# 0beqz/realism-effects

Hardware: AMD Instinct MI355X
Metric: Mpixels/s SSGI+denoise @4K steps=20; achieved HBM GB/s vs peak (higher is better)
Workload: dtype f32; 1 GPU; configs[2]: 3840x2160 (8.29 Mpixel) on one GPU, steps=20 refineSteps=5 denoiseIterations=1, K1+K2+2xK3+K4 per step; frame=3840x2160, tile_rows=2160, halo_rows=0, direct_light=True, half_store=rtz, uv_model=reference_gl, parallelism=single GPU

## Files before the change

realism-effects_amd/csrc/k1_ssgi.hip:

```cpp
#include "rfx_blocks.h"
#include "rfx_brdf.h"
#include "rfx_kernels.h"
#include "rfx_launch.h"

namespace {

constexpr int BASE = 16;
constexpr int K1_TH = 1;
typedef uint32_t k1_cell_t;
constexpr int K1_WAVES = 8;
constexpr int K1_COUNTERS = 64;
constexpr int K1_TABLE_CELLS = RFX_K1_TABLE_BYTES / (int)sizeof(k1_cell_t);
RFX_DEV uint32_t k1_half_toward(float v, bool up) {
    uint32_t h = rfx_f2h_rne(v) & 0xffffu;
    const float f = rfx_h2f((unsigned short)h);
    if (up ? (f < v) : (f > v)) {
        const bool neg = (h & 0x8000u) != 0;
        if (up) h = neg ? (h == 0x8000u ? 0x0001u : h - 1u) : h + 1u;
        else h = neg ? h + 1u : (h == 0x0000u ? 0x8001u : h - 1u);
    }
    return h;
}
RFX_DEV k1_cell_t k1_cell_pack(float mn, float mx) { return k1_half_toward(mn, false) | (k1_half_toward(mx, true) << 16); }
RFX_DEV float2 k1_cell_load(const k1_cell_t *t, unsigned int i) {
    const uint32_t v = *(const k1_cell_t *)((const char *)t + i);
    return make_float2(rfx_h2f((unsigned short)(v & 0xffffu)), rfx_h2f((unsigned short)(v >> 16)));
}

struct MarchCtx {
    const float *P;
    const float *viewz;
    const k1_cell_t *coarse;
    int coarse_w, cell_shift;
    unsigned int cell_xmask;
    int cell_xshift, cell_yshift;
    float rayDistance, thickness;
    int steps, refineSteps;
};

RFX_DEV float k1_div(float x, float w, float r) {
    const float q = x * r;
    return __builtin_fmaf(__builtin_fmaf(-w, q, x), r, q);
}
constexpr int PROJ_GENERAL = 0, PROJ_PERSPECTIVE = 1, PROJ_CENTRED = 2;
constexpr int PROJ_TABLE_POW2 = 4;
constexpr int k1_proj_kind(int proj) { return proj & 3; }
constexpr bool k1_table_pow2(int proj) { return (proj & PROJ_TABLE_POW2) != 0; }
template <int PROJ_T>
RFX_DEV float2 k1_project(const MarchCtx &m, float3 p) {
    constexpr int PROJ = k1_proj_kind(PROJ_T);
    float px, py, pw;
    if (PROJ == PROJ_CENTRED) {
        px = m.P[0] * p.x;
        py = m.P[5] * p.y;
        pw = -p.z;
    } else if (PROJ == PROJ_PERSPECTIVE) {
        px = m.P[0] * p.x + m.P[8] * p.z;
        py = m.P[5] * p.y + m.P[9] * p.z;
        pw = -p.z;
    } else {
        const float4 pc = rfx_mat_mul(m.P, p.x, p.y, p.z, 1.0f);
        px = pc.x; py = pc.y; pw = pc.w;
    }
    const float r = rfx_rcp(pw);
    return make_float2(__builtin_fmaf(k1_div(px, pw, r), 0.5f, 0.5f), __builtin_fmaf(k1_div(py, pw, r), 0.5f, 0.5f));
}

struct Tap {
    unsigned int idx;
    unsigned int cell;
};
template <bool P2>
RFX_DEV Tap k1_tap_at(const MarchCtx &m, const FrameDims &d, int xi, int yi) {
    Tap t;
    t.idx = (unsigned int)(__mul24(yi, d.W) + xi);
    if (P2) {
        const unsigned int a = (unsigned int)xi >> m.cell_xshift, b = (unsigned int)yi << m.cell_yshift;
        t.cell = (unsigned int)__builtin_amdgcn_bitop3_b32((int)a, (int)b, (int)m.cell_xmask, 0xE4);
    } else {
// ... 55 lines not shown
    if (need[0] | need[1]) {
        const unsigned int i0 = need[0] ? tap[0].idx : tap[1].idx, i1 = need[1] ? tap[1].idx : tap[0].idx;
        const float z0 = rfx_gather<float>(m.viewz, i0), z1 = rfx_gather<float>(m.viewz, i1);
        const float d0 = z0 - rays[0].pos.z, d1 = z1 - rays[1].pos.z;
        rays[0].live = (need[0] & (d0 >= 0.0f) & (d0 < m.thickness)) ? 0.0f : rays[0].live;
        rays[1].live = (need[1] & (d1 >= 0.0f) & (d1 < m.thickness)) ? 0.0f : rays[1].live;
    }
}
template <int PROJ>
RFX_DEV void k1_refine_pairs(const MarchCtx &m, const FrameDims &d, Ray (&rays)[2]) {
#pragma unroll
    for (int r = 0; r < 2; r++) {
        rays[r].dir = rays[r].dir * 0.5f;
        rays[r].pos = rays[r].pos + rays[r].dir * (rays[r].hit ? -1.0f : 0.0f);
    }
    for (int k = 0; k < m.refineSteps; k++) {
#pragma unroll
        for (int r = 0; r < 2; r++)
            if (rays[r].hit) rays[r].uv = k1_project<PROJ>(m, rays[r].pos);
        Tap tap[2];
        float2 mm[2];
        bool need[2], behind[2];
#pragma unroll
        for (int r = 0; r < 2; r++) tap[r] = k1_tap<k1_table_pow2(PROJ)>(m, d, rays[r].uv);
#pragma unroll
        for (int r = 0; r < 2; r++) {
            need[r] = rays[r].hit;
            behind[r] = false;
        }
#pragma unroll
        for (int r = 0; r < 2; r++) mm[r] = k1_cell_load(m.coarse, tap[r].cell);
#pragma unroll
        for (int r = 0; r < 2; r++) {
            const float h = rays[r].pos.z;
            const bool below = mm[r].y - h < 0.0f;
            const bool above = !below & (mm[r].x - h >= 0.0f);
            need[r] = need[r] & !(below | above);
            behind[r] = above;
        }
        float z[2];
#pragma unroll
        for (int r = 0; r < 2; r++) z[r] = need[r] ? rfx_gather<float>(m.viewz, tap[r].idx) : 0.0f;
#pragma unroll
        for (int r = 0; r < 2; r++) {
            if (need[r]) behind[r] = z[r] - rays[r].pos.z >= 0.0f;
            rays[r].dir = rays[r].dir * 0.5f;
            rays[r].pos = rays[r].pos + rays[r].dir * (rays[r].hit ? (behind[r] ? -1.0f : 1.0f) : 0.0f);
        }
    }
#pragma unroll
    for (int r = 0; r < 2; r++)
        if (rays[r].hit) rays[r].uv = k1_project<PROJ>(m, rays[r].pos);
}
RFX_DEV float k1_push(int dest_lane, float v) { return __int_as_float(__builtin_amdgcn_ds_permute(dest_lane << 2, __float_as_int(v))); }
RFX_DEV float k1_pull(int src_lane, float v) { return __int_as_float(__builtin_amdgcn_ds_bpermute(src_lane << 2, __float_as_int(v))); }
template <int PROJ>
RFX_DEV void k1_refine_packed(const MarchCtx &m, const FrameDims &d, Ray (&rays)[2], unsigned long long h0, unsigned long long h1, int n0, int n1) {
    const int lane = (int)__builtin_amdgcn_mbcnt_hi(~0u, __builtin_amdgcn_mbcnt_lo(~0u, 0u));
    const int rank0 = (int)__builtin_amdgcn_mbcnt_hi((unsigned int)(h0 >> 32), __builtin_amdgcn_mbcnt_lo((unsigned int)h0, 0u));
    const int rank1 = n0 + (int)__builtin_amdgcn_mbcnt_hi((unsigned int)(h1 >> 32), __builtin_amdgcn_mbcnt_lo((unsigned int)h1, 0u));
    const int dest0 = rays[0].hit ? rank0 : 63, dest1 = rays[1].hit ? rank1 : 63;
    const bool from0 = lane < n0, mine = lane < n0 + n1;
    float3 pos, dir;
#define K1_PACK(dst, field) { const float a = k1_push(dest0, rays[0].field), b = k1_push(dest1, rays[1].field); dst = from0 ? a : b; }
    K1_PACK(pos.x, pos.x) K1_PACK(pos.y, pos.y) K1_PACK(pos.z, pos.z) K1_PACK(dir.x, dir.x) K1_PACK(dir.y, dir.y) K1_PACK(dir.z, dir.z)
#undef K1_PACK
    dir = dir * 0.5f;
    pos = pos + dir * (mine ? -1.0f : 0.0f);
    float2 uv = make_float2(0.f, 0.f);
    for (int k = 0; k < m.refineSteps; k++) {
        if (mine) uv = k1_project<PROJ>(m, pos);
        const Tap tap = k1_tap<k1_table_pow2(PROJ)>(m, d, uv);
        const float2 mm = k1_cell_load(m.coarse, tap.cell);
        const float h = pos.z;
        const bool below = mm.y - h < 0.0f;
        const bool above = !below & (mm.x - h >= 0.0f);
        const bool need = mine & !(below | above);
        bool behind = above;
        const float z = need ? rfx_gather<float>(m.viewz, tap.idx) : 0.0f;
        if (need) behind = z - pos.z >= 0.0f;
        dir = dir * 0.5f;
        pos = pos + dir * (mine ? (behind ? -1.0f : 1.0f) : 0.0f);
    }
    if (mine) uv = k1_project<PROJ>(m, pos);
#define K1_UNPACK(val, f0, f1) { const float a = k1_pull(rank0, val), b = k1_pull(rank1, val); if (rays[0].hit) f0 = a; if (rays[1].hit) f1 = b; }
    K1_UNPACK(pos.x, rays[0].pos.x, rays[1].pos.x) K1_UNPACK(pos.y, rays[0].pos.y, rays[1].pos.y) K1_UNPACK(pos.z, rays[0].pos.z, rays[1].pos.z)
    K1_UNPACK(uv.x, rays[0].uv.x, rays[1].uv.x) K1_UNPACK(uv.y, rays[0].uv.y, rays[1].uv.y)
#undef K1_UNPACK
}
template <int PROJ>
RFX_DEV void k1_march_rays(const MarchCtx &m, const FrameDims &d, Ray (&rays)[2], float random_b) {
    const float scale = m.rayDistance / (float)m.steps;
    const bool started[2] = {rays[0].live != 0.0f, true};
#pragma unroll
    for (int r = 0; r < 2; r++) {
        rays[r].dir = rays[r].dir * scale;
        rays[r].uv = make_float2(0.f, 0.f);
    }
    const int split = min(m.steps, 9);
    int i = 1;
    for (; i < split && K1_ANY_LIVE(rays); i++) {
        const float t = (float)i + random_b - 0.5f;
        const float cs = 1.0f - rfx_exp2((t * t) * (-0.25f * 1.4426950408889634f));
        k1_march_step<PROJ, false>(m, d, rays, cs);
    }
    for (; i < m.steps && K1_ANY_LIVE(rays); i++) k1_march_step<PROJ, true>(m, d, rays, 1.0f);
#pragma unroll
    for (int r = 0; r < 2; r++) rays[r].hit = started[r] & (rays[r].live == 0.0f);
    if (m.refineSteps > 0) {
        const unsigned long long h0 = __ballot(rays[0].hit), h1 = __ballot(rays[1].hit);
        const int n0 = __popcll(h0), n1 = __popcll(h1);
// ... 267 lines not shown
        const float3 diffuseRay = (MIS && ems.isEnvSample) ? envMisDir : rfx_cosine_sample_hemisphere(viewNormal, rnd.x, rnd.y);
        diffuseRayDir = diffuseRay;
        const Angles ad = k1_angles(diffuseRay, vv, n);
        brdfD = k1_brdf_over_pdf_parts(mat, viewNormal, roughnessSq, true, NoV, ad, diffuseRay, pdfD);
        rays[0].dir = diffuseRay;
    }
    an = k1_angles(specularRay, vv, n);
    brdfS = k1_brdf_over_pdf_parts(mat, viewNormal, roughnessSq, isDiffuseSample, NoV, an, specularRay, pdfS);
    rays[1].live = 1.0f;
    rays[1].pos = viewPos;
    rays[1].dir = specularRay;
    if (STAGE == 2) {
        const float4 h0 = A.hits[2 * out_idx], h1 = A.hits[2 * out_idx + 1];
        rays[0].uv = make_float2(h0.x, h0.y);
        rays[1].uv = make_float2(h0.z, h0.w);
        rays[0].pos = make_float3(h1.x, h1.x, h1.x);
        rays[1].pos = make_float3(h1.y, h1.z, h1.w);
    } else {
        k1_march_rays<PROJ>(m, d, rays, rnd.z);
    }
    if (STAGE == 1) {
        A.hits[2 * out_idx] = make_float4(rays[0].uv.x, rays[0].uv.y, rays[1].uv.x, rays[1].uv.y);
        A.hits[2 * out_idx + 1] = make_float4(rays[0].pos.x, rays[1].pos.x, rays[1].pos.y, rays[1].pos.z);
        return;
    }

    float3 diffuseGI = make_float3(-1.0f, -1.0f, -1.0f);
    if (isDiffuseSample) diffuseGI = k1_shade<ENV, MIS>(d, A, mat, roughnessSq, rays[0], diffuseRayDir, true, brdfD, pdfD, ems) + dl;
    const float3 specularGI = k1_shade<ENV, MIS>(d, A, mat, roughnessSq, rays[1], specularRay, isDiffuseSample, brdfS, pdfS, ems) + dl;
    const float3 hitPos = rays[1].pos;

    float rayLength = 0.0f;
    if (!(hitPos.x > 10.0e8f)) {
        const float4 hw = rfx_mat_mul(C, hitPos.x, hitPos.y, hitPos.z, 1.0f);
        rayLength = rfx_length(make_float3(C[12], C[13], C[14]) - make_float3(hw.x, hw.y, hw.z));
    }
    if (p.mode == 0) {
        *outp = rfx_pack_two_vec4(make_float4(diffuseGI.x, diffuseGI.y, diffuseGI.z, mat.roughness),
                                  make_float4(specularGI.x, specularGI.y, specularGI.z, rayLength));
    } else {
        *outp = make_uint4(__float_as_uint(specularGI.x), __float_as_uint(specularGI.y), __float_as_uint(specularGI.z), rfx_pack_half2(rayLength, mat.roughness));
    }
}

template <int PROJ, bool ENV, bool MIS, int STAGE>
__global__ __launch_bounds__(64 * K1_WAVES) RFX_WAVES_PER_EU(ENV ? 1 : 8) void k1_ssgi_march(K1Args A) {
    __shared__ k1_cell_t s_cells[K1_TABLE_CELLS];
    if (STAGE != 2) {
        for (int i = threadIdx.x; i < A.cells_vec4; i += 64 * K1_WAVES) ((uint4 *)s_cells)[i] = ((const uint4 *)A.cells)[i];
        __syncthreads();
    }
    FrameDims d = A.dims;
    d.viol = 0;
    const int lane = threadIdx.x & 63;
    const unsigned int nbx = (unsigned int)(A.out_w + 63) / 64u, nby = (unsigned int)(A.y1 - A.y0 + K1_TH - 1) / (unsigned int)K1_TH, ntiles = nbx * nby;
    const unsigned int nq = min((unsigned int)K1_COUNTERS, gridDim.x);
    const unsigned int first = blockIdx.x % nq;
    unsigned int *counter = A.tile_counter + first * 32u;
    const auto k1_tile_of = [&](unsigned int n, unsigned int &bx, unsigned int &by) -> bool {
        const unsigned int tile = n * nq + first;
        by = tile / nbx;
        bx = tile - by * nbx;
        return tile < ntiles;
    };
    unsigned int n = 0;
    if (lane == 0) n = atomicAdd(counter, 1u);
    n = (unsigned int)__builtin_amdgcn_readfirstlane((int)n);
    unsigned int bx, by;
    while (k1_tile_of(n, bx, by)) {
        unsigned int next = 0;
        if (lane == 0) next = atomicAdd(counter, 1u);
        const int x = (int)bx * 64 + lane, y0 = A.y0 + (int)by * K1_TH;
#pragma unroll 1
        for (int r = 0; r < K1_TH; r++) {
            k1_ssgi_march_body<PROJ, ENV, MIS, STAGE>(RFX_KERNARGS_IN_LOOP(A), d, s_cells, x, y0 + r);
            RFX_WAVE_JOIN();
        }
        n = (unsigned int)__builtin_amdgcn_readfirstlane((int)next);
    }
    rfx_flush_violations(d);
}

__global__ __launch_bounds__(256) void k1_hit_mask(FrameDims d, int y0, int y1, TexView depth, TexViewW out, const float4 *hits, int allow_missed, unsigned int *mask) {
    const int x = blockIdx.x * 64 + threadIdx.x, y = y0 + blockIdx.y * 4 + threadIdx.y;
    d.viol = 0;
    if (x >= d.W || y >= y1) return;
    const float dp = ((const float *)depth.ptr)[rfx_xy_index(d, depth.row0, depth.rows, x, y)];
    if (dp == 1.0f) return;
    const size_t i = (size_t)rfx_local_row(d, out.row0, out.rows, y) * d.W + x;
    const float4 h0 = hits[2 * i], h1 = hits[2 * i + 1];
    const float u[2] = {h0.x, h0.z}, v[2] = {h0.y, h0.w}, px[2] = {h1.x, h1.y};
#pragma unroll
    for (int r = 0; r < 2; r++) {
        const bool missed = px[r] == 10.0e9f;
        if ((allow_missed || !missed) && u[r] >= 0.0f && u[r] <= 1.0f && v[r] >= 0.0f && v[r] <= 1.0f) {
            const int row = rfx_nearest_idx(v[r], d.fH, d.H), col = rfx_nearest_idx(u[r], d.fW, d.W);
            const unsigned int bit = 1u << rfx_block_of_col(col, d.W);
            if (!(mask[row] & bit)) atomicOr(&mask[row], bit);
        }
    }
}

template <int VEC>
__global__ __launch_bounds__(256) void k1_prepare(const float *depth, float *viewz, float2 *base, int W, int H, int base_w, float nearMulFar,
                                                   float farMinusNear, float cameraFar, float nearMinusFar, float cameraNear, int perspective,
                                                   unsigned char *fg, int fg_w) {
    static_assert(VEC == 1 || VEC == 4, "one texel or one aligned float4 per lane and row");
// ... 154 lines not shown
```

realism-effects_amd/csrc/k4_compose.hip:

```cpp
#include "k4_compose_texel.h"
#include "rfx_blocks.h"
#include "rfx_launch.h"

namespace {

template <bool WHOLE>
RFX_DEV void k4_compose_body(const K4Args &A, const FrameDims &d) {
    const int x = blockIdx.x * 64 + threadIdx.x;
    const int y = A.y0 + blockIdx.y * 4 + threadIdx.y;
    if (x >= d.W || y >= A.y1) return;
    const float u = rfx_frag_u(d.uv, x, y), v = rfx_frag_v(d.uv, y);
    const float *depthp = (const float *)A.depth.ptr;
    const float depth = depthp[rfx_xy_index(d, A.depth.row0, A.depth.rows, x, y)];
    {
        const int qx0 = x & ~1, qx1 = x | 1, qy0 = y & ~1, qy1 = y | 1;
        float dxa = depthp[rfx_xy_index(d, A.depth.row0, A.depth.rows, qx0, y)], dxb = depthp[rfx_xy_index(d, A.depth.row0, A.depth.rows, qx1, y)];
        float dya = depthp[rfx_xy_index(d, A.depth.row0, A.depth.rows, x, qy0)], dyb = depthp[rfx_xy_index(d, A.depth.row0, A.depth.rows, x, qy1)];
        if (depth == 1.0f && (fabsf(dxb - dxa) + fabsf(dyb - dya)) == 0.0f) {
            if (A.rgb_out) {
                const float4 keep = ((const float4 *)A.out.ptr)[(size_t)rfx_local_row(d, A.out.row0, A.out.rows, y) * d.W + x];
                float *r = A.rgb_out + ((size_t)y * d.W + x) * 3;
                r[0] = keep.x; r[1] = keep.y; r[2] = keep.z;
            }
            return;
        }
    }
    const Material mat = rfx_get_material<true>(((const uint4 *)A.gbuffer.ptr)[rfx_xy_index(d, A.gbuffer.row0, A.gbuffer.rows, x, y)]);
    float4 dgi = make_float4(0.f, 0.f, 0.f, 0.f), sgi;
    if (A.p.giSource) {
        const size_t gi = rfx_xy_index(d, A.gi0.row0, A.gi0.rows, x, y);
        if (A.p.inputType == 0) {
            dgi = ((const float4 *)A.gi0.ptr)[gi];
            sgi = ((const float4 *)A.gi1.ptr)[gi];
        } else {
            sgi = ((const float4 *)A.gi0.ptr)[gi];
        }
    } else if (A.p.inputType == 0) {
        dgi = rfx_fetch_h4_linear_fused<WHOLE>(A.gi0, d, u, v);
        sgi = rfx_fetch_h4_linear_fused<WHOLE>(A.gi1, d, u, v);
    } else {
        sgi = rfx_fetch_h4_linear_fused<WHOLE>(A.gi0, d, u, v);
    }
    float3 scene = make_float3(0.f, 0.f, 0.f);
    if (A.p.inputType == 2) {
        const float4 sc = ((const float4 *)A.scene.ptr)[rfx_xy_index(d, A.scene.row0, A.scene.rows, x, y)];
        scene = make_float3(sc.x, sc.y, sc.z);
    }
    const float4 o = k4_compose_texel(A.p, u, v, depth, mat, make_float3(dgi.x, dgi.y, dgi.z), make_float3(sgi.x, sgi.y, sgi.z), scene);
    ((float4 *)A.out.ptr)[(size_t)rfx_local_row(d, A.out.row0, A.out.rows, y) * d.W + x] = o;
    if (A.rgb_out) {
        float *r = A.rgb_out + ((size_t)y * d.W + x) * 3;
        r[0] = o.x; r[1] = o.y; r[2] = o.z;
    }
}

template <bool WHOLE>
__global__ __launch_bounds__(256) void k4_compose(K4Args A) {
    FrameDims d = A.dims;
    d.viol = 0;
    k4_compose_body<WHOLE>(A, d);
    rfx_flush_violations(d);
}

__global__ __launch_bounds__(256) void k5_final_compose(K5Args A) {
    FrameDims d = A.dims;
    d.viol = 0;
    const int x = blockIdx.x * 64 + threadIdx.x, y = A.y0 + blockIdx.y * 4 + threadIdx.y;
    if (x < d.W && y < A.y1) {
        const rfx_final_params &p = A.p;
        float4 o;
        const size_t gii = rfx_xy_index(d, A.gi.row0, A.gi.rows, x, y);
        const float4 gi = p.inputSource == 2 ? rfx_load_half4(((const uint2 *)A.gi.ptr)[gii]) : ((const float4 *)A.gi.ptr)[gii];
        if (p.isDebug) {
            o = gi;
        } else {
            const float depth = ((const float *)A.depth.ptr)[rfx_xy_index(d, A.depth.row0, A.depth.rows, x, y)];
            float3 c;
            if (depth == 1.0f) {
                const float4 sc = ((const float4 *)A.scene.ptr)[rfx_xy_index(d, A.scene.row0, A.scene.rows, x, y)];
                c = make_float3(sc.x, sc.y, sc.z);
            } else {
                c = make_float3(gi.x, gi.y, gi.z);
                if (p.fogMode) {
                    const float n_ = p.camera.near_, f_ = p.camera.far_;
                    const float viewZ = rfx_depth_to_view_z(depth, n_, f_, p.camera.isPerspective != 0) * 0.4f;
                    const float fd = -viewZ;
                    float ff;
                    if (p.fogMode == 2) {
                        ff = 1.0f - rfx_exp(((-p.fogDensity * p.fogDensity) * fd) * fd);
                    } else {
                        const float t = rfx_clamp((fd - p.fogNear) / (p.fogFar - p.fogNear), 0.0f, 1.0f);
                        ff = t * t * (3.0f - 2.0f * t);
                    }
                    c = rfx_mix(c, make_float3(p.fogColor[0], p.fogColor[1], p.fogColor[2]), ff);
                }
            }
            o = make_float4(c.x, c.y, c.z, 1.0f);
        }
        ((float4 *)A.out.ptr)[(size_t)rfx_local_row(d, A.out.row0, A.out.rows, y) * d.W + x] = o;
    }
    rfx_flush_violations(d);
}


struct K6Foot {
    int x0, x1, y0, y1;
    float wx, wy;
};
RFX_DEV K6Foot k6_footprint(const FrameDims &d, float u, float v) {
#pragma clang fp contract(off)
    const float cx = u * d.fW, cy = v * d.fH;
    const LinearCoord lx = rfx_linear_coord_fast(cx, d.fW - 0.5f), ly = rfx_linear_coord_fast(cy, d.fH - 0.5f);
    K6Foot f;
    f.x0 = lx.i0; f.y0 = ly.i0;
// ... 129 lines not shown
    if (live) {
        p.bits = p.rows == rows ? (p.bits | bits) : bits;
        p.rows = rows;
    }
}

__global__ __launch_bounds__(256) void k6_motion_blur_reach(K6Args A) {
#pragma clang fp contract(off)
    FrameDims d = A.dims;
    d.viol = 0;
    const int x = blockIdx.x * 64 + threadIdx.x, y = A.y0 + blockIdx.y * 4 + threadIdx.y;
    if (y >= A.y1) return;
    const bool in_frame = x < d.W;
    const int xc = min(x, d.W - 1);
    const float u = rfx_frag_u(d.uv, xc, y), v = rfx_frag_v(d.uv, y);
    K6Pending pend;
    pend.rows = -1; pend.bits = 0u;
    if (A.center_is_source) k6_name(A.reach_mask, pend, k6_footprint(d, u, v), d.W, in_frame);
    const float4 vel = rfx_gather<float4>(A.velocity, (unsigned int)__mul24(rfx_local_row(d, A.vel_row0, A.vel_rows, y), d.W) + (unsigned int)xc);
    const bool moved = in_frame && k6_moved(vel.x, vel.y);
    if (__ballot(moved) != 0) {
        const K6Streak s = k6_streak(A, u, v, vel.x, vel.y);
        for (int i = 0; i <= A.samples; i++) {
            const float2 tuv = k6_tap_uv(A, s, i);
            k6_name(A.reach_mask, pend, k6_footprint(d, tuv.x, tuv.y), d.W, moved);
        }
    }
    k6_flush_wave(A.reach_mask, pend, pend.rows >= 0);
    rfx_flush_violations(d);
}

}

hipError_t rfx_launch_k6(const K6Args &A, hipStream_t stream) {
    dim3 block(16, 16), grid((A.dims.W + 15) / 16, (A.y1 - A.y0 + 15) / 16);
    if (A.tiled) hipLaunchKernelGGL(k6_motion_blur_tiled, grid, block, 0, stream, A);
    else hipLaunchKernelGGL(k6_motion_blur, grid, block, 0, stream, A);
    return hipGetLastError();
}

hipError_t rfx_launch_k6_reach(const K6Args &A, hipStream_t stream) {
    dim3 block(64, 4), grid((A.dims.W + 63) / 64, (A.y1 - A.y0 + 3) / 4);
    hipLaunchKernelGGL(k6_motion_blur_reach, grid, block, 0, stream, A);
    return hipGetLastError();
}

hipError_t rfx_launch_k5(const K5Args &A, hipStream_t stream) {
    dim3 block(64, 4), grid((A.dims.W + 63) / 64, (A.y1 - A.y0 + 3) / 4);
    hipLaunchKernelGGL(k5_final_compose, grid, block, 0, stream, A);
    return hipGetLastError();
}

hipError_t rfx_launch_k4(const K4Args &A, hipStream_t stream) {
    dim3 block(64, 4), grid((A.dims.W + 63) / 64, (A.y1 - A.y0 + 3) / 4);
    rfx_with_bool(rfx_views_whole(A.dims.H, A.gi0, A.gi1), [&](auto wh) { hipLaunchKernelGGL(k4_compose<decltype(wh)::value>, grid, block, 0, stream, A); });
    return hipGetLastError();
}
```

realism-effects_amd/csrc/rfx_api.hip:

```cpp
#include <hip/hip_runtime.h>
#include <stdio.h>
#include <stdlib.h>
#include <string.h>
#include <string>
#include "../../include/rfx.h"
#include "rfx_kernels.h"
#include "rfx_launch.h"

#include "rfx_ctx.h"

thread_local std::string g_create_err;

#define RFX_ENTER(c) hipSetDevice((c)->device)
static hipEvent_t prof_event(rfx_ctx *c) {
    hipEvent_t e = nullptr;
    if (!c->prof_free.empty()) { e = c->prof_free.back(); c->prof_free.pop_back(); return e; }
    return hipEventCreate(&e) == hipSuccess ? e : nullptr;
}
static void prof_recycle(rfx_ctx *c) {
    for (const rfx_ctx::ProfRec &r : c->prof_recs) { c->prof_free.push_back(r.a); c->prof_free.push_back(r.b); }
    c->prof_recs.clear();
}
struct ProfScope {
    rfx_ctx *c;
// ... 639 lines not shown
        A.maxEnvMapMipLevel = c->env ? (float)(lg + 1) : 0.0f;
    }
    A.hits = stage != 0 ? c->hits : nullptr;
    return any;
}

static int k1_prepass(rfx_ctx *c, const K1Args &A) {
    if (c->depth_external) {
        ProfScope prof(c, RFX_PROF_K1_PREPASS, c->stream);
        HIPCHK(c, rfx_launch_k1_prepare(A, c->stream));
    } else {
        if (c->depth_event_set) HIPCHK(c, hipStreamWaitEvent(c->prep_stream, c->ev_depth, 0));
        if (c->k1_event_set) HIPCHK(c, hipStreamWaitEvent(c->prep_stream, c->ev_k1_done, 0));
        {
            ProfScope prof(c, RFX_PROF_K1_PREPASS, c->prep_stream);
            HIPCHK(c, rfx_launch_k1_prepare(A, c->prep_stream));
        }
        HIPCHK(c, hipEventRecord(c->ev_prep_done, c->prep_stream));
        HIPCHK(c, hipStreamWaitEvent(c->stream, c->ev_prep_done, 0));
    }
    c->fg_cur ^= 1;
    c->fg_gen = c->depth_gen;
    return RFX_OK;
}

static int ssgi_draw(rfx_ctx *c, const rfx_ssgi_params *p, int stage) {
    int rc = ssgi_validate(c, p);
    if (rc) return rc;
    const rfx_k1_table_plan T = rfx_k1_table(c->W, c->H);
    const int base = rfx_k1_base_cell(), coarse_w = (c->W + base - 1) / base, coarse_h = (c->H + base - 1) / base;
    if ((rc = k1_scratch(c, T, coarse_w, coarse_h))) return rc;
    if ((rc = k1_hand_over(c, stage))) return rc;
    K1Args A;
    const bool any = k1_args(c, p, stage, T, coarse_w, coarse_h, A);
    if (stage != 2 && (rc = k1_prepass(c, A))) return rc;
    if (any && stage == 2) HIPCHK(c, hipMemsetAsync(c->k1_tiles, 0, 64 * 128, c->stream));
    if (any) {
        ProfScope prof(c, RFX_PROF_K1_MARCH, c->stream);
        HIPCHK(c, rfx_launch_k1(A, stage, c->stream));
    }
    HIPCHK(c, hipEventRecord(c->ev_k1_done, c->stream));
    c->k1_event_set = true;
    c->hits_traced = stage == 1;
    if (stage == 1) { c->trace_y0 = A.y0; c->trace_y1 = any ? A.y1 : A.y0; c->trace_missed = p->missedRays; c->trace_scaled = ssgi_resolution_scale(p) != 1.0f; }
    return RFX_OK;
}

int rfx_internal_k1_table(int W, int H, struct rfx_k1_table_plan *out) {
    *out = rfx_k1_table(W, H);
    return RFX_OK;
}
int rfx_internal_k3_tile(int W, int H, float radius, int inputIsTemporal, int textureCount, struct rfx_k3_tile_plan *out) {
    *out = rfx_k3_tile((float)W, (float)H, radius, inputIsTemporal != 0, textureCount);
    return RFX_OK;
}

static int hit_mask_scratch(rfx_ctx *c, int ranks) {
    if (ranks < 1) ranks = 1;
    if (!c->hit_mask_dev || c->hit_mask_ranks < ranks) {
        if (c->hit_mask_dev) {
            HIPCHK(c, hipStreamSynchronize(c->stream));
            if (c->comm_stream) HIPCHK(c, hipStreamSynchronize(c->comm_stream));
            hipFree(c->hit_mask_dev); hipHostFree(c->hit_mask_host); c->hit_mask_dev = nullptr; c->hit_mask_host = nullptr;
        }
        const size_t words = (size_t)(2 * ranks + 2) * c->H;
        hipError_t e = hipMalloc((void **)&c->hit_mask_dev, words * sizeof(unsigned int));
        if (e == hipSuccess) e = hipHostMalloc((void **)&c->hit_mask_host, words * sizeof(unsigned int), hipHostMallocDefault);
        if (e != hipSuccess) return fail(c, RFX_ENOMEM, "rfx_ssgi_hit_mask: scratch", e);
        c->hit_mask_ranks = ranks;
    }
    return RFX_OK;
}

int rfx_internal_hit_mask_enqueue(rfx_ctx *c, int ranks) {
    if (!c->hits || !c->hits_traced) return fail(c, RFX_ESTATE, "rfx_gather_history_rows / rfx_ssgi_hit_mask: no rfx_ssgi_trace of this frame is waiting for its shade");
    if (c->trace_scaled) return fail(c, RFX_EUNSUPPORTED, "rfx_ssgi_hit_mask / rfx_gather_history_rows: the last rfx_ssgi_trace ran with resolutionScale != 1");
    RFX_ENTER(c);
    int rc = hit_mask_scratch(c, ranks);
    if (rc) return rc;
    HIPCHK(c, hipMemsetAsync(c->hit_mask_dev, 0, (size_t)c->H * sizeof(unsigned int), c->stream));
    if (c->trace_y1 > c->trace_y0)
        HIPCHK(c, rfx_launch_k1_hit_mask(dims(c), c->trace_y0, c->trace_y1, view(c, RFX_TEX_DEPTH), wview(c, RFX_TEX_SSGI), c->hits, c->trace_missed != 0, c->hit_mask_dev, c->stream));
    return RFX_OK;
}

static int hit_mask_read_back(rfx_ctx *c, unsigned int *row_mask) {
    const size_t bytes = (size_t)c->H * sizeof(unsigned int);
    HIPCHK(c, hipMemcpyAsync(c->hit_mask_host, c->hit_mask_dev, bytes, hipMemcpyDeviceToHost, c->stream));
    HIPCHK(c, hipStreamSynchronize(c->stream));
    if (row_mask) memcpy(row_mask, c->hit_mask_host, bytes);
    return RFX_OK;
}

int rfx_ssgi_hit_mask(rfx_ctx *c, unsigned int *row_mask, int rows) {
    if (!c || !row_mask) return RFX_EINVAL;
    if (rows != c->H) return fail(c, RFX_EINVAL, "rfx_ssgi_hit_mask: one word per frame row (rows == height)");
    int rc = rfx_internal_hit_mask_enqueue(c, 1);
    if (rc) return rc;
    return hit_mask_read_back(c, row_mask);
}

int rfx_ssgi_hit_rows(rfx_ctx *c, int *row_lo, int *row_hi) {
    if (!c || !row_lo || !row_hi) return RFX_EINVAL;
    int rc = rfx_internal_hit_mask_enqueue(c, 1);
    if (rc || (rc = hit_mask_read_back(c, nullptr))) return rc;
    int lo = 0x7fffffff, hi = -1;
// ... 345 lines not shown
```

realism-effects_amd/csrc/rfx_ctx.h:

```cpp
#pragma once
#include <hip/hip_runtime.h>
#include <stdio.h>
#include <string>
#include <vector>
#include "../../include/rfx.h"

struct Slot {
    void *ptr = nullptr;
    bool owned = false;
    int row0 = 0, rows = 0;
    size_t texel = 0;
    int width = 0;
    bool uploaded = false;
    void *back = nullptr;
    bool back_filled = false;
};

struct rfx_ctx {
    int device = 0;
    int W = 0, H = 0, tile_y0 = 0, tile_rows = 0, halo = 0;
    hipStream_t own_stream = nullptr, stream = nullptr;
    hipEvent_t ev0 = nullptr, ev1 = nullptr;
    unsigned int *halo_violations = nullptr;
    float *viewz = nullptr;
// ... 8 lines not shown
    hipStream_t prep_stream = nullptr;
    hipEvent_t ev_depth = nullptr, ev_k1_done = nullptr, ev_prep_done = nullptr;
    bool depth_event_set = false, k1_event_set = false, depth_external = false;
    int win_y0 = 0, win_y1 = 0x7fffffff;
    int blur_armed = -1;
    int uv_model = RFX_UV_REFERENCE_GL;
    float2 *coarse = nullptr;
    unsigned int *cells = nullptr;
    unsigned int *k1_tiles = nullptr;
    int n_cu = 0;
    unsigned char *fg_tiles = nullptr;
    size_t fg_stride = 0;
    int fg_w = 0, fg_cur = 0;
    unsigned long long depth_gen = 1, fg_gen = 0;
    float4 *env = nullptr;
    float *env_marginal = nullptr, *env_conditional = nullptr;
    float env_sum_whole = 1.0f, env_sum_decimal = 0.0f;
    int env_w = 0, env_h = 0, env_levels = 0;
    unsigned int env_off[16] = {0};
    Slot slots[RFX_TEX_COUNT];
    void *comm = nullptr;
    bool comm_owned = false;
    int comm_rank = 0, comm_nranks = 1;
    hipStream_t comm_stream = nullptr;
    hipEvent_t ev_draws = nullptr, ev_comm = nullptr;
    bool comm_pending = false;
    hipStream_t upload_stream = nullptr;
    hipEvent_t ev_staged = nullptr, ev_frame_done = nullptr;
    hipEvent_t ev_batch[2] = {nullptr, nullptr};
    unsigned int flips = 0;
    unsigned long long *peer_flags = nullptr;
    void **peer_table_dev = nullptr;
    unsigned long long *peer_status_dev = nullptr, *peer_status_host = nullptr;
    std::vector<void *> peer_mapped;
    hipEvent_t ev_peer_release = nullptr;
    bool peer_release_pending = false;
    int peer_n = 0, peer_rank = 0, peer_tex = -1;
    unsigned long long peer_epoch = 0;
    struct ProfRec { int kind; hipEvent_t a, b; };
    bool profiling = false;
    std::vector<ProfRec> prof_recs;
    std::vector<hipEvent_t> prof_free;
    std::string err;
};
void rfx_comm_release(rfx_ctx *c);
int rfx_ensure_streams(rfx_ctx *c);
int rfx_comm_begin(rfx_ctx *c);
int rfx_comm_end(rfx_ctx *c);
void rfx_peer_release(rfx_ctx *c);
extern "C" int rfx_internal_hit_mask_enqueue(rfx_ctx *c, int ranks);
extern "C" int rfx_internal_blur_reach_enqueue(rfx_ctx *c, const rfx_motion_blur_params *p, int ranks);
extern "C" int rfx_internal_k1_table(int W, int H, struct rfx_k1_table_plan *out);
extern "C" int rfx_internal_k3_tile(int W, int H, float radius, int inputIsTemporal, int textureCount, struct rfx_k3_tile_plan *out);

extern thread_local std::string g_create_err;

static inline size_t texel_bytes(int id) {
    switch (id) {
    case RFX_TEX_DEPTH: return 4;
    case RFX_TEX_BLUE_NOISE: return 4;
    case RFX_TEX_COMPOSE_RGB: return 12;
    case RFX_TEX_DENOISE_A0: case RFX_TEX_DENOISE_A1: case RFX_TEX_DENOISE_B0: case RFX_TEX_DENOISE_B1: case RFX_TEX_FBCOPY_F16: return 8;
    default: return 16;
    }
}

static inline int fail(rfx_ctx *c, int code, const char *what, hipError_t e = hipSuccess) {
    char buf[512];
    if (e != hipSuccess) {
        snprintf(buf, sizeof buf, "%s: %s", what, hipGetErrorString(e));
        (void)hipGetLastError();
    } else snprintf(buf, sizeof buf, "%s", what);
    if (c) c->err = buf;
    else g_create_err = buf;
    return code;
}
#define HIPCHK(c, call)                                              \
    do {                                                             \
        hipError_t e__ = (call);                                     \
        if (e__ != hipSuccess) return fail(c, RFX_EDEVICE, #call, e__); \
    } while (0)
```

realism-effects_amd/csrc/rfx_launch.h:

```cpp
#pragma once
#include <hip/hip_runtime.h>
#include <type_traits>

constexpr int RFX_K1_TABLE_BYTES = 36864;
struct rfx_k1_table_plan { int cell_shift, cells_w, cells_h, pitch, pitch_log2, pow2, vec4; };
inline rfx_k1_table_plan rfx_k1_table(int W, int H) {
    const auto k1_table = [&](int shift, bool pow2, int &cw, int &ch, int &pitch, int &pitch_log2) {
        cw = (W + (1 << shift) - 1) >> shift;
        ch = (H + (1 << shift) - 1) >> shift;
        pitch = cw;
        pitch_log2 = 0;
        if (pow2) {
            pitch_log2 = shift;
            while ((1 << pitch_log2) < cw) pitch_log2++;
            pitch = 1 << pitch_log2;
        }
        return (size_t)((pitch * ch + 3) / 4) * 16;
    };
    rfx_k1_table_plan t;
    t.pow2 = 0;
    for (t.cell_shift = 4;; t.cell_shift++) {
        if (k1_table(t.cell_shift, false, t.cells_w, t.cells_h, t.pitch, t.pitch_log2) <= (size_t)RFX_K1_TABLE_BYTES || t.cell_shift >= 12) break;
    }
    int cw, ch, pitch, pl2;
    if (k1_table(t.cell_shift, true, cw, ch, pitch, pl2) <= (size_t)RFX_K1_TABLE_BYTES) {
        t.pow2 = 1;
        t.pitch = pitch;
        t.pitch_log2 = pl2;
    }
    t.vec4 = (t.pitch * t.cells_h + 3) / 4;
    return t;
}

constexpr int RFX_K3_TW = 64, RFX_K3_TH = 8;
constexpr int K3_LDS_MAX = 80 * 1024;
struct rfx_k3_tile_plan { int Rx, Ry, LW, LH, pitch, skip; size_t lds_bytes; int tiled; };
inline rfx_k3_tile_plan rfx_k3_tile(float fW, float fH, float radius, bool temporal, int textureCount) {
    constexpr int TW = RFX_K3_TW, TH = RFX_K3_TH;
    rfx_k3_tile_plan t;
    const float aspect = fW / fH;
    const float rx = radius * fmaxf(1.0f, aspect), ry = radius * fmaxf(1.0f, 1.0f / aspect);
    const float SLACK = 4e-3f;
    const auto k3_apron = [&](float r) {
        const int a = temporal ? (int)floorf(r + 0.5f + SLACK) : (int)floorf(r + SLACK) + 1;
        return a < 1 ? 1 : a;
    };
    t.Rx = k3_apron(rx);
    t.Ry = k3_apron(ry);
    t.LW = TW + 2 * t.Rx;
    t.LH = TH + 2 * t.Ry;
    t.skip = 0;
    t.pitch = t.LW <= TW + 8 ? TW + 8 : t.LW <= TW + 10 ? TW + 10 : t.LW <= TW + 12 ? TW + 12 : t.LW <= TW + 16 ? TW + 16 : t.LW <= TW + 32 ? TW + 32 : 0;
    t.lds_bytes = (size_t)t.pitch * t.LH * (16 + 4 + 2 * (temporal ? 16 : 8));
    if (temporal && textureCount == 2 && t.pitch == t.LW && t.pitch != 0) {
        const float q = ((float)t.Ry - 0.5f - SLACK) / ry;
        const int X = (int)floorf(0.5f + rx * sqrtf(fmaxf(0.0f, 1.0f - q * q)) + SLACK);
        int skip = t.Rx - X;
        if (skip > 4) skip = 4;
        const int ntex = t.pitch * t.LH;
        while (skip > 0 && ((ntex - 2 * skip) & 3) != 0) skip--;
        if (skip > 0) {
            t.skip = skip;
            t.lds_bytes = 16 + (size_t)(ntex - 2 * skip) * (4 + 16 + 32) + (size_t)skip * 32;
        }
    }
    t.tiled = radius >= 0.0f && t.pitch != 0 && t.lds_bytes <= (size_t)K3_LDS_MAX;
    return t;
}

template <class... V>
inline bool rfx_views_whole(int H, const V &...v) {
    return ((v.ptr == nullptr || (v.row0 == 0 && v.rows == H)) && ...);
}

template <class F>
inline void rfx_with_bool(bool b, F &&f) {
    b ? f(std::true_type{}) : f(std::false_type{});
}
template <int... Vs, class F>
inline bool rfx_with_int(int x, F &&f) {
    return ((x == Vs && (f(std::integral_constant<int, Vs>{}), true)) || ...);
}

template <auto Kernel, class T, class F>
inline T rfx_per_device(F &&get) {
// ... 9 lines not shown
```

Baseline: 6536 Mpixels/s.

## Pack K1 depth cells as bf16 bounds and process two rows per K4 thread

The K1 min/max depth cells move from fp16 with directed rounding to truncated bfloat16 bounds. Unpacking becomes a shift or mask instead of a half-to-float conversion, and packing becomes cheap bit arithmetic. The K4 compose kernel now handles two vertically adjacent pixels per thread. It gets the horizontal depth neighbour via a lane shuffle instead of extra global loads, and splits loading from finishing so loads can be issued early. Host helpers for cell pack/unpack are added for testing; bf16 has coarser mantissa precision, so the bounds are looser and may cause extra refinement work in the march.

```diff
diff --git a/realism-effects_amd/csrc/k1_ssgi.hip b/realism-effects_amd/csrc/k1_ssgi.hip
--- a/realism-effects_amd/csrc/k1_ssgi.hip
+++ b/realism-effects_amd/csrc/k1_ssgi.hip
@@ -11,20 +11,10 @@
 constexpr int K1_WAVES = 8;
 constexpr int K1_COUNTERS = 64;
 constexpr int K1_TABLE_CELLS = RFX_K1_TABLE_BYTES / (int)sizeof(k1_cell_t);
-RFX_DEV uint32_t k1_half_toward(float v, bool up) {
-    uint32_t h = rfx_f2h_rne(v) & 0xffffu;
-    const float f = rfx_h2f((unsigned short)h);
-    if (up ? (f < v) : (f > v)) {
-        const bool neg = (h & 0x8000u) != 0;
-        if (up) h = neg ? (h == 0x8000u ? 0x0001u : h - 1u) : h + 1u;
-        else h = neg ? h + 1u : (h == 0x0000u ? 0x8001u : h - 1u);
-    }
-    return h;
-}
-RFX_DEV k1_cell_t k1_cell_pack(float mn, float mx) { return k1_half_toward(mn, false) | (k1_half_toward(mx, true) << 16); }
+RFX_DEV k1_cell_t k1_cell_pack(float mn, float mx) { return rfx_k1_cell_pack_bits(__float_as_uint(mn), __float_as_uint(mx)); }
 RFX_DEV float2 k1_cell_load(const k1_cell_t *t, unsigned int i) {
     const uint32_t v = *(const k1_cell_t *)((const char *)t + i);
-    return make_float2(rfx_h2f((unsigned short)(v & 0xffffu)), rfx_h2f((unsigned short)(v >> 16)));
+    return make_float2(__uint_as_float(rfx_k1_cell_min_bits(v)), __uint_as_float(rfx_k1_cell_max_bits(v)));
 }
 
 struct MarchCtx {
@@ -186,11 +176,12 @@
     for (int r = 0; r < 2; r++)
         if (rays[r].hit) rays[r].uv = k1_project<PROJ>(m, rays[r].pos);
 }
+RFX_DEV int k1_lane() { return (int)__builtin_amdgcn_mbcnt_hi(~0u, __builtin_amdgcn_mbcnt_lo(~0u, 0u)); }
 RFX_DEV float k1_push(int dest_lane, float v) { return __int_as_float(__builtin_amdgcn_ds_permute(dest_lane << 2, __float_as_int(v))); }
 RFX_DEV float k1_pull(int src_lane, float v) { return __int_as_float(__builtin_amdgcn_ds_bpermute(src_lane << 2, __float_as_int(v))); }
 template <int PROJ>
 RFX_DEV void k1_refine_packed(const MarchCtx &m, const FrameDims &d, Ray (&rays)[2], unsigned long long h0, unsigned long long h1, int n0, int n1) {
-    const int lane = (int)__builtin_amdgcn_mbcnt_hi(~0u, __builtin_amdgcn_mbcnt_lo(~0u, 0u));
+    const int lane = k1_lane();
     const int rank0 = (int)__builtin_amdgcn_mbcnt_hi((unsigned int)(h0 >> 32), __builtin_amdgcn_mbcnt_lo((unsigned int)h0, 0u));
     const int rank1 = n0 + (int)__builtin_amdgcn_mbcnt_hi((unsigned int)(h1 >> 32), __builtin_amdgcn_mbcnt_lo((unsigned int)h1, 0u));
     const int dest0 = rays[0].hit ? rank0 : 63, dest1 = rays[1].hit ? rank1 : 63;
@@ -564,7 +555,7 @@
     }
     FrameDims d = A.dims;
     d.viol = 0;
-    const int lane = threadIdx.x & 63;
+    const int lane = k1_lane();
     const unsigned int nbx = (unsigned int)(A.out_w + 63) / 64u, nby = (unsigned int)(A.y1 - A.y0 + K1_TH - 1) / (unsigned int)K1_TH, ntiles = nbx * nby;
     const unsigned int nq = min((unsigned int)K1_COUNTERS, gridDim.x);
     const unsigned int first = blockIdx.x % nq;
diff --git a/realism-effects_amd/csrc/k4_compose.hip b/realism-effects_amd/csrc/k4_compose.hip
--- a/realism-effects_amd/csrc/k4_compose.hip
+++ b/realism-effects_amd/csrc/k4_compose.hip
@@ -4,48 +4,66 @@
 
 namespace {
 
+struct K4Foot {
+    uint2 t00, t10, t01, t11;
+    float wx, wy;
+};
+struct K4In {
+    uint4 g;
+    K4Foot l0, l1;
+    float4 n0, n1;
+    float4 sc;
+};
 template <bool WHOLE>
-RFX_DEV void k4_compose_body(const K4Args &A, const FrameDims &d) {
-    const int x = blockIdx.x * 64 + threadIdx.x;
-    const int y = A.y0 + blockIdx.y * 4 + threadIdx.y;
-    if (x >= d.W || y >= A.y1) return;
-    const float u = rfx_frag_u(d.uv, x, y), v = rfx_frag_v(d.uv, y);
-    const float *depthp = (const float *)A.depth.ptr;
-    const float depth = depthp[rfx_xy_index(d, A.depth.row0, A.depth.rows, x, y)];
+RFX_DEV K4Foot k4_foot_load(const TexView &t, const FrameDims &d, float u, float v) {
+    float cx, cy;
     {
-        const int qx0 = x & ~1, qx1 = x | 1, qy0 = y & ~1, qy1 = y | 1;
-        float dxa = depthp[rfx_xy_index(d, A.depth.row0, A.depth.rows, qx0, y)], dxb = depthp[rfx_xy_index(d, A.depth.row0, A.depth.rows, qx1, y)];
-        float dya = depthp[rfx_xy_index(d, A.depth.row0, A.depth.rows, x, qy0)], dyb = depthp[rfx_xy_index(d, A.depth.row0, A.depth.rows, x, qy1)];
-        if (depth == 1.0f && (fabsf(dxb - dxa) + fabsf(dyb - dya)) == 0.0f) {
-            if (A.rgb_out) {
-                const float4 keep = ((const float4 *)A.out.ptr)[(size_t)rfx_local_row(d, A.out.row0, A.out.rows, y) * d.W + x];
-                float *r = A.rgb_out + ((size_t)y * d.W + x) * 3;
-                r[0] = keep.x; r[1] = keep.y; r[2] = keep.z;
-            }
-            return;
-        }
-    }
-    const Material mat = rfx_get_material<true>(((const uint4 *)A.gbuffer.ptr)[rfx_xy_index(d, A.gbuffer.row0, A.gbuffer.rows, x, y)]);
+#pragma clang fp contract(off)
+        cx = u * d.fW;
+        cy = v * d.fH;
+    }
+    const LinearCoord lx = rfx_linear_coord_fast(cx, d.fW - 0.5f), ly = rfx_linear_coord_fast(cy, d.fH - 0.5f);
+    const int x1 = min(lx.i0 + 1, d.W - 1), y1 = min(ly.i0 + 1, d.H - 1);
+    const unsigned int r0 = (unsigned int)__mul24(rfx_view_row<WHOLE>(d, t, ly.i0), d.W), r1 = (unsigned int)__mul24(rfx_view_row<WHOLE>(d, t, y1), d.W);
+    K4Foot f;
+    f.t00 = rfx_gather<uint2>(t.ptr, r0 + lx.i0); f.t10 = rfx_gather<uint2>(t.ptr, r0 + x1);
+    f.t01 = rfx_gather<uint2>(t.ptr, r1 + lx.i0); f.t11 = rfx_gather<uint2>(t.ptr, r1 + x1);
+    f.wx = lx.w; f.wy = ly.w;
+    return f;
+}
+RFX_DEV float4 k4_foot_blend(const K4Foot &f) { return rfx_bilerp_half_rgba(f.t00, f.t10, f.t01, f.t11, f.wx, f.wy); }
+
+template <bool WHOLE>
+RFX_DEV void k4_load(const K4Args &A, const FrameDims &d, int x, int y, float u, float v, K4In &in) {
+    in.g = ((const uint4 *)A.gbuffer.ptr)[rfx_xy_index(d, A.gbuffer.row0, A.gbuffer.rows, x, y)];
+    if (A.p.giSource) {
+        const size_t gi = rfx_xy_index(d, A.gi0.row0, A.gi0.rows, x, y);
+        in.n0 = ((const float4 *)A.gi0.ptr)[gi];
+        if (A.p.inputType == 0) in.n1 = ((const float4 *)A.gi1.ptr)[gi];
+    } else {
+        in.l0 = k4_foot_load<WHOLE>(A.gi0, d, u, v);
+        if (A.p.inputType == 0) in.l1 = k4_foot_load<WHOLE>(A.gi1, d, u, v);
+    }
+    if (A.p.inputType == 2) in.sc = ((const float4 *)A.scene.ptr)[rfx_xy_index(d, A.scene.row0, A.scene.rows, x, y)];
+}
+RFX_DEV void k4_finish(const K4Args &A, const FrameDims &d, int x, int y, float u, float v, float depth, const K4In &in) {
+    const Material mat = rfx_get_material<true>(in.g);
     float4 dgi = make_float4(0.f, 0.f, 0.f, 0.f), sgi;
     if (A.p.giSource) {
-        const size_t gi = rfx_xy_index(d, A.gi0.row0, A.gi0.rows, x, y);
         if (A.p.inputType == 0) {
-            dgi = ((const float4 *)A.gi0.ptr)[gi];
-            sgi = ((const float4 *)A.gi1.ptr)[gi];
+            dgi = in.n0;
+            sgi = in.n1;
         } else {
-            sgi = ((const float4 *)A.gi0.ptr)[gi];
+            sgi = in.n0;
         }
     } else if (A.p.inputType == 0) {
-        dgi = rfx_fetch_h4_linear_fused<WHOLE>(A.gi0, d, u, v);
-        sgi = rfx_fetch_h4_linear_fused<WHOLE>(A.gi1, d, u, v);
+        dgi = k4_foot_blend(in.l0);
+        sgi = k4_foot_blend(in.l1);
     } else {
-        sgi = rfx_fetch_h4_linear_fused<WHOLE>(A.gi0, d, u, v);
+        sgi = k4_foot_blend(in.l0);
     }
     float3 scene = make_float3(0.f, 0.f, 0.f);
-    if (A.p.inputType == 2) {
-        const float4 sc = ((const float4 *)A.scene.ptr)[rfx_xy_index(d, A.scene.row0, A.scene.rows, x, y)];
-        scene = make_float3(sc.x, sc.y, sc.z);
-    }
+    if (A.p.inputType == 2) scene = make_float3(in.sc.x, in.sc.y, in.sc.z);
     const float4 o = k4_compose_texel(A.p, u, v, depth, mat, make_float3(dgi.x, dgi.y, dgi.z), make_float3(sgi.x, sgi.y, sgi.z), scene);
     ((float4 *)A.out.ptr)[(size_t)rfx_local_row(d, A.out.row0, A.out.rows, y) * d.W + x] = o;
     if (A.rgb_out) {
@@ -53,13 +71,50 @@
         r[0] = o.x; r[1] = o.y; r[2] = o.z;
     }
 }
+RFX_DEV void k4_keep(const K4Args &A, const FrameDims &d, int x, int y) {
+    if (!A.rgb_out) return;
+    const float4 keep = ((const float4 *)A.out.ptr)[(size_t)rfx_local_row(d, A.out.row0, A.out.rows, y) * d.W + x];
+    float *r = A.rgb_out + ((size_t)y * d.W + x) * 3;
+    r[0] = keep.x; r[1] = keep.y; r[2] = keep.z;
+}
+
+template <bool WHOLE>
+RFX_DEV unsigned int k4_compose_body(const K4Args &A, const FrameDims &d) {
+    const int x = blockIdx.x * 64 + threadIdx.x;
+    const int ya = (A.y0 & ~1) + blockIdx.y * 8 + 2 * threadIdx.y, yb = ya + 1;
+    const bool in_a = ya >= A.y0 && ya < A.y1, in_b = yb < A.y1;
+    if (x >= d.W || !(in_a | in_b)) return 0u;
+    const float *depthp = (const float *)A.depth.ptr;
+    const float da = depthp[rfx_xy_index(d, A.depth.row0, A.depth.rows, x, ya)], db = depthp[rfx_xy_index(d, A.depth.row0, A.depth.rows, x, yb)];
+    FrameDims d0 = d, d1 = d;
+    const float ua = rfx_frag_u(d.uv, x, ya), ub = rfx_frag_u(d.uv, x, yb), va = rfx_frag_v(d.uv, ya), vb = rfx_frag_v(d.uv, yb);
+    const bool partner = (x ^ 1) < d.W, odd = (x & 1) != 0;
+    const float sa = __shfl_xor(da, 1), sb = __shfl_xor(db, 1);
+    const float pa = partner ? sa : da, pb = partner ? sb : db;
+    const float fy = fabsf(db - da);
+    const bool keep_a = da == 1.0f && (fabsf(odd ? da - pa : pa - da) + fy) == 0.0f;
+    const bool keep_b = db == 1.0f && (fabsf(odd ? db - pb : pb - db) + fy) == 0.0f;
+    const bool draw_a = in_a && !keep_a, draw_b = in_b && !keep_b;
+    if (in_a && keep_a) k4_keep(A, d0, x, ya);
+    if (in_b && keep_b) k4_keep(A, d1, x, yb);
+    K4In ia, ib;
+    if (draw_a) {
+        k4_load<WHOLE>(A, d0, x, ya, ua, va, ia);
+        k4_finish(A, d0, x, ya, ua, va, da, ia);
+    }
+    if (draw_b) {
+        k4_load<WHOLE>(A, d1, x, yb, ub, vb, ib);
+        k4_finish(A, d1, x, yb, ub, vb, db, ib);
+    }
+    return (unsigned int)(in_a && d0.viol) + (unsigned int)(in_b && d1.viol);
+}
 
 template <bool WHOLE>
 __global__ __launch_bounds__(256) void k4_compose(K4Args A) {
     FrameDims d = A.dims;
     d.viol = 0;
-    k4_compose_body<WHOLE>(A, d);
-    rfx_flush_violations(d);
+    const unsigned int viol = k4_compose_body<WHOLE>(A, d);
+    if (viol && d.halo_violations) atomicAdd(d.halo_violations, viol);
 }
 
 __global__ __launch_bounds__(256) void k5_final_compose(K5Args A) {
@@ -295,7 +350,7 @@
 }
 
 hipError_t rfx_launch_k4(const K4Args &A, hipStream_t stream) {
-    dim3 block(64, 4), grid((A.dims.W + 63) / 64, (A.y1 - A.y0 + 3) / 4);
+    dim3 block(64, 4), grid((A.dims.W + 63) / 64, (A.y1 - (A.y0 & ~1) + 7) / 8);
     rfx_with_bool(rfx_views_whole(A.dims.H, A.gi0, A.gi1), [&](auto wh) { hipLaunchKernelGGL(k4_compose<decltype(wh)::value>, grid, block, 0, stream, A); });
     return hipGetLastError();
 }
diff --git a/realism-effects_amd/csrc/rfx_api.hip b/realism-effects_amd/csrc/rfx_api.hip
--- a/realism-effects_amd/csrc/rfx_api.hip
+++ b/realism-effects_amd/csrc/rfx_api.hip
@@ -715,6 +715,24 @@
 }
 int rfx_internal_k3_tile(int W, int H, float radius, int inputIsTemporal, int textureCount, struct rfx_k3_tile_plan *out) {
     *out = rfx_k3_tile((float)W, (float)H, radius, inputIsTemporal != 0, textureCount);
+    return RFX_OK;
+}
+
+int rfx_internal_k1_cell_pack(const float *mn, const float *mx, unsigned int *cells, int n) {
+    for (int i = 0; i < n; i++) {
+        uint32_t a, b;
+        memcpy(&a, &mn[i], 4);
+        memcpy(&b, &mx[i], 4);
+        cells[i] = rfx_k1_cell_pack_bits(a, b);
+    }
+    return RFX_OK;
+}
+int rfx_internal_k1_cell_unpack(const unsigned int *cells, float *mn, float *mx, int n) {
+    for (int i = 0; i < n; i++) {
+        const uint32_t a = rfx_k1_cell_min_bits(cells[i]), b = rfx_k1_cell_max_bits(cells[i]);
+        memcpy(&mn[i], &a, 4);
+        memcpy(&mx[i], &b, 4);
+    }
     return RFX_OK;
 }
 
diff --git a/realism-effects_amd/csrc/rfx_ctx.h b/realism-effects_amd/csrc/rfx_ctx.h
--- a/realism-effects_amd/csrc/rfx_ctx.h
+++ b/realism-effects_amd/csrc/rfx_ctx.h
@@ -84,6 +84,8 @@
 extern "C" int rfx_internal_blur_reach_enqueue(rfx_ctx *c, const rfx_motion_blur_params *p, int ranks);
 extern "C" int rfx_internal_k1_table(int W, int H, struct rfx_k1_table_plan *out);
 extern "C" int rfx_internal_k3_tile(int W, int H, float radius, int inputIsTemporal, int textureCount, struct rfx_k3_tile_plan *out);
+extern "C" int rfx_internal_k1_cell_pack(const float *mn, const float *mx, unsigned int *cells, int n);
+extern "C" int rfx_internal_k1_cell_unpack(const unsigned int *cells, float *mn, float *mx, int n);
 
 extern thread_local std::string g_create_err;
 
diff --git a/realism-effects_amd/csrc/rfx_launch.h b/realism-effects_amd/csrc/rfx_launch.h
--- a/realism-effects_amd/csrc/rfx_launch.h
+++ b/realism-effects_amd/csrc/rfx_launch.h
@@ -1,5 +1,6 @@
 #pragma once
 #include <hip/hip_runtime.h>
+#include <stdint.h>
 #include <type_traits>
 
 constexpr int RFX_K1_TABLE_BYTES = 36864;
@@ -31,6 +32,18 @@
     t.vec4 = (t.pitch * t.cells_h + 3) / 4;
     return t;
 }
+
+__host__ __device__ inline uint32_t rfx_k1_cell_bound(uint32_t bits, bool up) {
+    const uint32_t hi = bits >> 16;
+    if ((bits & 0x7fffffffu) > 0x7f800000u) return hi | 0x0040u;
+    const bool neg = (bits >> 31) != 0;
+    return hi + (uint32_t)(((bits & 0xffffu) != 0u) & (neg != up));
+}
+__host__ __device__ inline uint32_t rfx_k1_cell_pack_bits(uint32_t mn_bits, uint32_t mx_bits) {
+    return rfx_k1_cell_bound(mn_bits, false) | (rfx_k1_cell_bound(mx_bits, true) << 16);
+}
+__host__ __device__ inline uint32_t rfx_k1_cell_min_bits(uint32_t cell) { return cell << 16; }
+__host__ __device__ inline uint32_t rfx_k1_cell_max_bits(uint32_t cell) { return cell & 0xffff0000u; }
 
 constexpr int RFX_K3_TW = 64, RFX_K3_TH = 8;
 constexpr int K3_LDS_MAX = 80 * 1024;
```

Measured after the change: 6580 Mpixels/s (median of 6 runs). About the same (+0.7%).
